# NorESMhub/BLOM

Hardware: AMD Instinct MI355X
Metric: simulated-days/sec (higher is better)
Workload: dtype f64; 1 GPU; channel 208x512x53 as 1 tile(s) of 208x512x53 along i, 1 tile per GPU, isopyc_bulkml/remap/geopotential/uc/enscon, ntr=3 (TKE, length-scale slot, ideal age: the reference default build), baclin=900s batrop=18s lstep=50; config 2's step (phy/mod_blom_step.F90:96-253: init_fluxes, tmsmt1, cmnfld2, difest_isobml [the whole routine: diffusivities estimated every step (NorESM defaults incl. rhsctp; the; physics=full, forcing=default, spinup_steps=0

## Files before the change

blom_amd/csrc/blomgpu_internal.h:

```cpp
#pragma once
#include <hip/hip_runtime.h>
#include <cstdint>
#include <string>
#include <unordered_map>
#include <vector>
#include "exp_libm.h"

#define NBDY 4

#ifdef BLOM_HOSTEMU
#define WAIT_VMCNT0() ((void)0)
#else
#define WAIT_VMCNT0() asm volatile("s_waitcnt vmcnt(0)" ::: "memory")
#endif

#define BLOM_REAL_FIELDS(X)                                                              \
                                                                          \
  X(u, 2 * K) X(v, 2 * K) X(dp, 2 * K) X(dpu, 2 * K) X(dpv, 2 * K) X(temp, 2 * K)        \
  X(saln, 2 * K) X(sigma, 2 * K) X(uflx, 2 * K) X(vflx, 2 * K) X(utflx, 2 * K)           \
  X(vtflx, 2 * K) X(usflx, 2 * K) X(vsflx, 2 * K)                                        \
  X(p, K + 1) X(pu, K + 1) X(pv, K + 1) X(phi, K + 1) X(cau, K) X(cav, K)                \
  X(ubflxs, 3) X(vbflxs, 3) X(ub, 2) X(vb, 2) X(pb, 2) X(pbu, 2) X(pbv, 2)               \
  X(ubflxs_p, 2) X(vbflxs_p, 2) X(pb_p, 1) X(pbu_p, 1) X(pbv_p, 1) X(ubcors_p, 1)        \
  X(vbcors_p, 1) X(sealv, 1)                                                             \
// ... 164 lines not shown
struct BtGlobal;
struct TileTable {
  int npx = 0, npy = 0, itdm = 0, nranks = 0;
  std::vector<int> i0, ii;
  std::vector<int> j0, jj;
  std::vector<int> rank;
  void ew_neighbours(int px, int py, bool periodic, int *west, int *east) const;
  bool tensor_product() const;
};
const char *tiletable_build(int npx, int npy, int itdm, int jtdm, const int *i0_pe, const int *ii_pe, const int *j0_pe,
                            const int *jj_pe, TileTable *out);
struct Tiling {
  int npx = 1, npy = 1;
  int px = 0, py = 0;
  const TileTable *tab = nullptr;
  TileGroup *group = nullptr;
  RcclComm *rccl = nullptr;
  bool multi() const { return npx * npy > 1 || rccl != nullptr; }
};

struct StepState {
  bool in_sequence = false;
  bool defer_checks = false;
  bool remap_handed_over = false;
  bool pbcor1_handed_over = false;
  bool pbcor2_handed_over = false;
  bool pbcor2_dp_in_wk = false;
  bool fluxes_lean = false;
  bool fluxes_zeroed = false;
  bool mom_early_done = false;
  bool convec_col_ahead = false;
  bool cmn_on_side = false;
  bool diapfl_mom_on_side = false, updtrc_on_side = false;
  bool pscan_done_ahead = false;
};

struct blomgpu_ctx {
  std::string expcnf = "channel";
  bool csdiag = false;
  int cnsvdi = 0;
  int cppm_compat = 1;
  int cppm_limiting = 2;
  int ale_method = 102, ale_upper_bndr_ord = 6, ale_lower_bndr_ord = 4, ale_tracer_limiting = 203, ale_velocity_limiting = 203;
  bool ale_tracer_pc_upper = true, ale_tracer_pc_lower = false, ale_velocity_pc_upper = true, ale_velocity_pc_lower = false;
  bool ale_density_pc_upper = false, ale_density_pc_lower = false;
  int ale_regrid_method = 2, ale_k_range_plevel = 1;
  double ale_regrid_nudge_ts = 86400., ale_stab_fac_limit = .75, ale_dpvar_fac = .75, ale_smooth_diff_max = 50000.;
  int ale_dktzu = 4, ale_dktzl = 2;
  double ale_dpmin_interior = .1 * 9806.;
  int ndiff_rec_per_face = 0;
  int ndiff_surface_align = 1;
  double rm0 = 1.2, rm5 = 0., niwgf = 0., niwbf = .35, niwlf = .5;
  std::string mlrttp = "constant";
  double trxday = 0., srxday = 0., trxdpt = 1., srxdpt = 1., trxlim = 1.5, srxlim = .5, sref = 34.65, area = 0., xmi = 0.;
  int lmi[5] = {11, 12, 1, 2, 3};
  bool aptflx = false, apsflx = false, ditflx = false, disflx = false, srxbal = false;
  int ntda = 0;
  double swamxd = 200., brine_mlbase_frac = 0.;
  int mlrmth = 1;
  double eddtra_ce = .06, tau_mlr = 86400., tau_growing_hbl = 300., tau_decaying_hbl = 86400., tau_growing_hml = 3600.,
         tau_decaying_hml = 259200., lfmin = 5.e3, mlbl_max_ratio = 3., eddtra_cl = .25, mstar = .5, nstar = .066, wpup_min = 1.e-3;
  double egc = 0., eggam = 200., eglsmn = 4000., egmndf = 0., egmxdf = 1500., egidfq = 1., rhiscf = 0., ri0 = 1.2, tkepf = 0.;
  double bdml_logc = 0.;
  int eddf2d = 0, edsprs = 1, edanis = 0, redi3d = 0, rhsctp = 0, edfsmo = 0;
  int edritp_opt = 2, edwmth_opt = 1;
  bool full_physics = false;
// ... 135 lines not shown
int st_xcsum(blomgpu_ctx *, const double *a, int itype, double *sum);
int st_xcsum_dev(blomgpu_ctx *, const double *a, int itype, int slot, double **sums_dev);
int st_thermf(blomgpu_ctx *, int m, int n, int mm, int nn, int k1m, int k1n);
int st_niw_ke_tendency(blomgpu_ctx *, int m, int mm);
int st_difest_isobml_pre(blomgpu_ctx *, int m, int n, int mm, int nn);
int st_difest_isobml(blomgpu_ctx *, int m, int n, int mm, int nn);
int st_budget_sums(blomgpu_ctx *, int ncall, int n, int nn);
int st_barotp(blomgpu_ctx *, int m, int n, int mm, int nn, int k1m, int k1n);
int st_eddtra(blomgpu_ctx *, int m, int n, int mm, int nn, int k1m, int k1n);
int st_eddtra_ale(blomgpu_ctx *, int m, int n, int mm, int nn, int k1m, int k1n);
int st_cppm(blomgpu_ctx *, int m, int n, int mm, int nn, int k1m, int k1n);
int st_init_cppm(blomgpu_ctx *);
int st_mxlayr_tail(blomgpu_ctx *, int nn, int k1n);
int ctx_err_words(blomgpu_ctx *);
int ctx_check_errors(blomgpu_ctx *);
int st_kfpla_halo(blomgpu_ctx *, int n);
int st_cmnfld1(blomgpu_ctx *, int m, int n, int mm, int nn, int k1m, int k1n);
int st_cmnfld2(blomgpu_ctx *, int m, int n, int mm, int nn, int k1m, int k1n);
int diapfl_column3_launch(blomgpu_ctx *, int n, int nn, int *errflag);
#define R_BASE(ntr) (8 + 3 * (ntr))
#define R_DP(ntr) (R_BASE(ntr) + 0)
#define R_T(ntr) (R_BASE(ntr) + 1)
#define R_S(ntr) (R_BASE(ntr) + 2)
#define R_TR(ntr, nt) (R_BASE(ntr) + 3 + (nt))
int st_ale_vdifft(blomgpu_ctx *, int m, int n, int mm, int nn, int k1m, int k1n);
int st_ale_vdiffm(blomgpu_ctx *, int m, int n, int mm, int nn, int k1m, int k1n);
int st_ale_forcing(blomgpu_ctx *, int m, int n, int mm, int nn, int k1m, int k1n);
int st_cmnfld_bfsqi_ale(blomgpu_ctx *, int m, int n, int mm, int nn, int k1m, int k1n);
int st_ale_regrid_remap(blomgpu_ctx *, int m, int n, int mm, int nn, int k1m, int k1n);
void ale_free(blomgpu_ctx *);
int ale_check_deferred(blomgpu_ctx *);
int st_mxlayr(blomgpu_ctx *, int m, int n, int mm, int nn, int k1m, int k1n);
int st_mom_pupv(blomgpu_ctx *, int off, int lo, int hi);
int st_convec_velocity(blomgpu_ctx *, int nn);
int launch_dpudpv(blomgpu_ctx *, int off, int flags);
int remap_tile_launch(blomgpu_ctx *, int n, int mm, int nn, int tsel, bool fold);
int pbcor_tile_launch(blomgpu_ctx *, int which, int m, int offc, int offf, int from_remap);
int launch_pscan(blomgpu_ctx *, int off, int lo, int hi_off);
int st_xctilr(blomgpu_ctx *, double *base, int l1, int ld, int mh, int nh, int itype);
int st_xctilr_arctic_multi(blomgpu_ctx *, int nf, double *const *ptrs, const int *nlevs, const int *mhs, const int *nhs,
                           const int *itypes);
int st_xctilr_multi(blomgpu_ctx *, int nf, double *const *ptrs, const int *nlevs, int mh, int nh, const int *itypes);
int st_crc(blomgpu_ctx *, const double *base, int nlev, int itype, unsigned *crc);
int st_crc_strips(blomgpu_ctx *, double *base, int nlev, int itype, unsigned *out, int cap, int *l0, int *ns);
int ctx_locate_ptr(const blomgpu_ctx *, const double *p, size_t *offset);
int rccl_xctilr(blomgpu_ctx *, double *base, int nlev, int mhl, int nhl);
int rccl_barotp_replicated(blomgpu_ctx *, int m, int n, int mm, int nn, int k1m, int k1n);
blomgpu_ctx *bt_global_ctx(const blomgpu_ctx *);
struct RcclLanded {
  const double *from_west = nullptr, *from_east = nullptr;
  int has_w = 0, has_e = 0, per = 0, mhl = 0, nhl = 0, nlev = 0;
  double *send_west = nullptr, *send_east = nullptr;
  int prepacked = 0;
};
int rccl_xctilr_multi_ex(blomgpu_ctx *, double *const *fields, int nf, int nlev, int mhl, int nhl, RcclLanded *landed);
int rccl_xctilr_multi(blomgpu_ctx *, double *const *fields, int nf, int nlev, int mhl, int nhl);

__device__ inline void xcd_block(unsigned &bx, unsigned &by) {
  const unsigned gx = gridDim.x, n = gx * gridDim.y;
  const unsigned lin = blockIdx.y * gx + blockIdx.x;
  const unsigned x = lin & 7u, s = lin >> 3;
  const unsigned q = n >> 3, r = n & 7u;
  const unsigned nl = x * q + (x < r ? x : r) + s;
  bx = nl % gx;
  by = nl / gx;
}

// ... 18 lines not shown
```

blom_amd/csrc/stage_barotp.hip:

```cpp
#include "blomgpu_internal.h"

#define ONEM 9806.

#define THREAD_IJ(V)                                                       \
  const int t_ = blockIdx.x * blockDim.x + threadIdx.x;                    \
  if (t_ >= (V).nplane) return;                                            \
  const int i = t_ % (V).ni - (NBDY - 1), j = t_ / (V).ni - (NBDY - 1);    \
  const size_t c = t_

__global__ void k_bt_bounds(const DevView *__restrict__ Vp, int m, int nn) {
  const DevView &V = *Vp;
  THREAD_IJ(V);
  if (j < 1 || j > V.jj || i < 1 || i > V.ii) return;
  const size_t np = V.nplane, om = c + (size_t)(m - 1) * np;
  if (V.m[I_iu][c]) {
    const double pbu = V.f[F_pbu][om];
    V.f[F_uglue][c] = V.P.cwbdts * exp_libm(1. - pbu / (V.P.cwbdls * ONEM));
    double mx = 0., mn = 0.;
    for (int k0 = 0; k0 < V.kk; k0 += COLUMN_U) {
      double a0[COLUMN_U];
#pragma unroll
      for (int q = 0; q < COLUMN_U; q++) a0[q] = V.f[F_u][c + (size_t)((k0 + q < V.kk ? k0 + q : V.kk - 1) + nn) * np];
#pragma unroll
      for (int q = 0; q < COLUMN_U; q++)
// ... 243 lines not shown
  const int i = t % V.ni - (NBDY - 1), j = t / V.ni - (NBDY - 1);
  if (i < 0 || i > V.ii + 1 || j < V.jj || j > V.jj + 2) return;
  const size_t c = t, on = (size_t)(n - 1) * V.nplane;
  double q = V.f[F_umaxb][c]; V.f[F_umaxb][c] = V.f[F_uminb][c]; V.f[F_uminb][c] = q;
  q = V.f[F_xixp][c + on]; V.f[F_xixp][c + on] = V.f[F_xixm][c + on]; V.f[F_xixm][c + on] = q;
  const int ilo = V.itdm / 2 - V.i0 + 1;
  if (j > V.jj || i >= (ilo > 0 ? ilo : 0)) {
    q = V.f[F_vmaxb][c]; V.f[F_vmaxb][c] = V.f[F_vminb][c]; V.f[F_vminb][c] = q;
    q = V.f[F_xiyp][c + on]; V.f[F_xiyp][c + on] = V.f[F_xiym][c + on]; V.f[F_xiym][c + on] = q;
  }
}

int bt_pair_halo(blomgpu_ctx *c, int set);
bool bt_phase_usable(blomgpu_ctx *c);
int bt_phase_launch(blomgpu_ctx *c, int m, int n, int ml, int nl, double woa, double wob, double wna, double wnb, int lll0,
                    int last, int src, int *src_out, int *ml_out, int *nl_out);
int bt_phase_check(blomgpu_ctx *c);
int bt_overlap_usable(blomgpu_ctx *c);
int bt_block_mode(blomgpu_ctx *c);
int bt_block_launch(blomgpu_ctx *c, int mode, int m, int n, int ml, int nl, const int *ph_last, const double (*ph_w)[4], int src,
                    int *src_out, int *ml_out, int *nl_out);
int bt_pair_launch(blomgpu_ctx *c, int m, int n, int ml, int nl, const double *wo, const double *wm, const double *wn,
                   int do_odd, int do_even, int src, int tsel, RcclLanded *rim);
int bt_pair_halo_landed(blomgpu_ctx *c, int set, RcclLanded *landed);

int st_barotp_bounds(blomgpu_ctx *c, int m, int nn) {
  hipLaunchKernelGGL(k_bt_bounds, plane_grid(c->h, 1, 64), dim3(64), 0, c->stream, c->d, m, nn);
  return 0;
}
int st_barotp_on(blomgpu_ctx *c, int m, int n, int mm, int nn, int k1m, int k1n, bool with_bounds);
int st_barotp(blomgpu_ctx *c, int m, int n, int mm, int nn, int k1m, int k1n) {
  TimeScope ts(c, "barotp");
  if (c->tiling.rccl && c->bt_global) return rccl_barotp_replicated(c, m, n, mm, nn, k1m, k1n);
  return st_barotp_on(c, m, n, mm, nn, k1m, k1n, true);
}
int st_barotp_on(blomgpu_ctx *c, int m, int n, int mm, int nn, int k1m, int k1n, bool with_bounds) {
  (void)mm; (void)k1m; (void)k1n;
  const DevView &h = c->h;
  const size_t np = h.nplane;
  const int ii = h.ii, jj = h.jj, lstep = h.P.lstep;
  if (lstep < 2 || lstep % 2) return ctx_fail(c, "barotp: lstep must be even (phy/mod_time.F90:137-139)");
  const dim3 g = plane_grid(h), b(256);
  if (with_bounds) hipLaunchKernelGGL(k_bt_bounds, plane_grid(h, 1, 64), dim3(64), 0, c->stream, c->d, m, nn);
  hipLaunchKernelGGL(k_bt_pvtrop_old, g, b, 0, c->stream, c->d, n);
  hipLaunchKernelGGL(k_bt_pvtrop, g, b, 0, c->stream, c->d, n);
  struct { int f, lev, nh, it; } hl[] = {
      {F_uglue, 0, 2, 3}, {F_utotn, 0, 2, 13}, {F_umaxb, 0, 2, 3}, {F_uminb, 0, 2, 3},
      {F_vglue, 0, 2, 4}, {F_vtotn, 0, 2, 14}, {F_vmaxb, 0, 2, 4}, {F_vminb, 0, 2, 4},
      {F_pvtrop, n - 1, 3, 2}, {F_pgfxm, n - 1, 2, 13}, {F_xixp, n - 1, 2, 3}, {F_xixm, n - 1, 2, 3},
      {F_pgfym, n - 1, 2, 14}, {F_xiyp, n - 1, 2, 4}, {F_xiym, n - 1, 2, 4}};
  for (int nhw = 2; nhw <= 3; nhw++) {
    double *ptrs[16];
    int nl[16], it[16], nf = 0;
    for (auto &x : hl)
      if (x.nh == nhw) { ptrs[nf] = h.f[x.f] + (size_t)x.lev * np; nl[nf] = 1; it[nf] = x.it; nf++; }
    if (int rc = st_xctilr_multi(c, nf, ptrs, nl, 1, nhw, it)) return rc;
  }

  if (h.nreg == 2) hipLaunchKernelGGL(k_bt_arctic_swap, g, b, 0, c->stream, c->d, n);
  if (int rc = ctx_err_words(c)) return rc;
  c->bt_restart = true;
  int lll0 = 1, ml = 1, nl = 2, set = 0;
  double woa = 0., wob = 0., wna = 0., wnb = 0.;
  if (c->barotp_fused && h.nreg != 2 && bt_block_mode(c)) {
    int ph_last[5];
    double ph_w[5][4];
    for (int nb = 1; nb <= 5; nb++) {
// ... 145 lines not shown
```

blom_amd/csrc/stage_convec.hip:

```cpp
#include "blomgpu_internal.h"
#include "eos.h"
#include "diapfl_common.h"

#define PLANE_IJ(V)                                                        \
  unsigned bx_, by_;                                                       \
  xcd_block(bx_, by_);                                                     \
  const int t_ = bx_ * blockDim.x + threadIdx.x;                           \
  (void)by_;                                                               \
  if (t_ >= (V).nplane) return;                                            \
  const int i = t_ % (V).ni - (NBDY - 1), j = t_ / (V).ni - (NBDY - 1);    \
  const size_t c = t_;                                                     \
  (void)i; (void)j; (void)c

#define MAXTR 64
enum { CV_UN = 0 };

__global__ __launch_bounds__(64) void k_convec_column(const DevView *__restrict__ Vp, int n, int nn, int *errflag) {
  const DevView &V = *Vp;
  PLANE_IJ(V);
  if (j < 1 || j > V.jj || i < 1 || i > V.ii || !V.m[I_ip][c]) return;
  const int kk = V.kk, ntr = V.ntr;
  const size_t np = V.nplane;
  const double epsilp = 1.e-12;
  gd_t ttem = V.f[F_temp] + c + (size_t)nn * np - np, ssal = V.f[F_saln] + c + (size_t)nn * np - np;
  gd_t delp = V.f[F_dp] + c + (size_t)nn * np - np, dens = V.f[F_sigma] + c + (size_t)nn * np - np;
  gcd_t densr = V.f[F_sigmar] + c - np;
  gd_t trc = V.f[F_trc] + c + (size_t)nn * np - np;
  const size_t ntl = (size_t)2 * kk * np;
#define TT(k) ttem[(size_t)(k) * np]
#define SS(k) ssal[(size_t)(k) * np]
#define DP(k) delp[(size_t)(k) * np]
#define DN(k) dens[(size_t)(k) * np]
#define DR(k) densr[(size_t)(k) * np]
#define TR(nt, k) trc[(size_t)(nt) * ntl + (size_t)(k) * np]
  double tdps, sdps, dps, ttmp, stmp, dtmp, q = 0.;
// ... 141 lines not shown
        k = kmix;
        while (dn2 < DR(k)) {
          if (k == 3) break;
          k = k - 1;
        }
        mix_tracers(true, d2, kfpl, kmix, q, 2, k);
        dps = 0.;
        for (int kz = kfpl; kz <= kmix; kz++) {
          dps = dps + DP(kz);
          DP(kz) = 0.;
        }
        kfpl = k;
        TT(kfpl) = ttmp; SS(kfpl) = stmp; DN(kfpl) = dn2; DP(kfpl) = dps;
        for (k = kfpl + 1; k <= kmix; k++) {
          const double dr = DR(k);
          TT(k) = ttmp;
          DN(k) = dr;
          SS(k) = eosd::sofsig(V.P, dr, ttmp);
        }
      }
    }
  }
  *kfpla = kfpl;
  column_scan(V.f[F_p][c], delp + np, V.f[F_p] + c, np, kk);
#undef TT
#undef SS
#undef DP
#undef DN
#undef DR
#undef TR
}

template <int NSINGLE>
__global__ __launch_bounds__(64) void k_convec_velocity(const DevView *__restrict__ Vp, int nn) {
  const DevView &V = *Vp;
  PLANE_IJ(V);
  if (j < 1 || j > V.jj || i < 1 || i > V.ii) return;
  const bool isv = by_ == 1;
  if (!V.m[isv ? I_iv : I_iu][c]) return;
  const int kk = V.kk;
  const size_t np = V.nplane, cm = isv ? c - V.ni : c - 1;
  gd_t vel = V.f[isv ? F_v : F_u] + c + (size_t)nn * np - np;
  gcd_t po = V.f[isv ? F_pv : F_pu] + c - np;
  gcd_t p = V.f[F_p] - np;
  gd_t un = WK(V, CV_UN + (isv ? 1 : 0)) + c - np;
  const double pbot = po[(size_t)(kk + 1) * np];
#define CV_U 8
#define CV_B 6
  int ko = 1;
  double po_lo = 0., po_hi = po[(size_t)2 * np];
  double v_cur = vel[(size_t)1 * np], v_nxt = vel[(size_t)(kk >= 2 ? 2 : 1) * np];
  double po_nx = kk >= 2 ? po[(size_t)3 * np] : 1.e300;
  double pn_lo = 0.;
  for (int k0 = 1; k0 <= kk; k0 += CV_U) {
    double a0[CV_U], a1[CV_U];
#pragma unroll
    for (int u = 0; u < CV_U; u++) {
      const int kq = k0 + u <= kk ? k0 + u : kk;
      a0[u] = p[c + (size_t)(kq + 1) * np]; a1[u] = p[cm + (size_t)(kq + 1) * np];
    }
#pragma unroll
    for (int u = 0; u < CV_U; u++) {
      const int kn = k0 + u;
      if (kn > kk) break;
      const double pn_hi = .5 * (fmin2(pbot, a0[u]) + fmin2(pbot, a1[u]));
      double r;
      if (pn_hi - pn_lo == 0.) {
        r = 0.;
      } else {
        double udpn = 0.;
        int nmv = 0;
        while (pn_hi > po_hi) {
          if (NSINGLE >= 1000 || nmv < NSINGLE) {
            nmv++;
            udpn = udpn + v_cur * (po_hi - fmax2(po_lo, pn_lo));
            ko = ko + 1;
            po_lo = po_hi;
            po_hi = ko <= kk ? po_nx : 1.e300;
            v_cur = v_nxt;
            v_nxt = vel[(size_t)(ko + 1 <= kk ? ko + 1 : kk) * np];
            po_nx = ko + 1 <= kk ? po[(size_t)(ko + 2) * np] : 1.e300;
          } else {
            double w[CV_B], q[CV_B];
#pragma unroll
            for (int b = 0; b < CV_B; b++) {
              const int kv = ko + 2 + b;
              w[b] = vel[(size_t)(kv <= kk ? kv : kk) * np];
              q[b] = po[(size_t)(kv <= kk ? kv + 1 : kk + 1) * np];
            }
#pragma unroll
            for (int b = 0; b < CV_B; b++)
              if (pn_hi > po_hi) {
                udpn = udpn + v_cur * (po_hi - fmax2(po_lo, pn_lo));
                ko = ko + 1;
                po_lo = po_hi;
                po_hi = ko <= kk ? po_nx : 1.e300;
                v_cur = v_nxt;
                v_nxt = w[b];
                po_nx = ko + 1 <= kk ? q[b] : 1.e300;
              }
          }
        }
        r = (udpn + v_cur * (pn_hi - fmax2(po_lo, pn_lo))) / (pn_hi - pn_lo);
      }
      un[(size_t)kn * np] = r;
      pn_lo = pn_hi;
    }
  }
  for (int k0 = 1; k0 <= kk; k0 += CV_U) {
    double a0[CV_U];
#pragma unroll
    for (int u = 0; u < CV_U; u++) a0[u] = un[(size_t)(k0 + u <= kk ? k0 + u : kk) * np];
#pragma unroll
    for (int u = 0; u < CV_U; u++)
      if (k0 + u <= kk) vel[(size_t)(k0 + u) * np] = a0[u];
  }
}

#define CVF_W 6
__global__ __launch_bounds__(64) void k_convec_velocity_flat(const DevView *__restrict__ Vp, int nn) {
  const DevView &V = *Vp;
  PLANE_IJ(V);
  __shared__ double s_pn[CVF_W][64], s_vel[CVF_W][64], s_po[CVF_W][64];
  if (j < 1 || j > V.jj || i < 1 || i > V.ii) return;
  const bool isv = by_ == 1;
  if (!V.m[isv ? I_iv : I_iu][c]) return;
  const int kk = V.kk, ln = threadIdx.x;
  const size_t np = V.nplane, cm = isv ? c - V.ni : c - 1;
  gd_t vel = V.f[isv ? F_v : F_u] + c + (size_t)nn * np - np;
  gcd_t po = V.f[isv ? F_pv : F_pu] + c - np;
  gcd_t p = V.f[F_p] - np;
  gd_t un = WK(V, CV_UN + (isv ? 1 : 0)) + c - np;
  const double pbot = po[(size_t)(kk + 1) * np];
  int ko = 1, of = 2, so_r = 2 % CVF_W, so_w = 2 % CVF_W;
  double po_lo = 0., po_hi = po[(size_t)2 * np], v_cur = vel[(size_t)1 * np], v_nx = 0., q_nx = 0.;
  bool hv_o = false;
  int kn = 1, nf = 1, sn_r = 1 % CVF_W, sn_w = 1 % CVF_W;
  double pn_lo = 0., pn_hi = 0., udpn = 0.;
  bool hv_n = false;
  while (kn <= kk) {
    if (__any(!hv_n || !hv_o)) {
      double a0[CVF_W], a1[CVF_W], w[CVF_W], q[CVF_W];
#pragma unroll
      for (int b = 0; b < CVF_W; b++) {
        const int lv = nf + b <= kk ? nf + b : kk, m = of + b <= kk ? of + b : kk;
        a0[b] = p[c + (size_t)(lv + 1) * np]; a1[b] = p[cm + (size_t)(lv + 1) * np];
        w[b] = vel[(size_t)m * np]; q[b] = po[(size_t)(m + 1) * np];
      }
// ... 45 lines not shown
    for (int u = 0; u < CV_U; u++) a0[u] = un[(size_t)(k0 + u <= kk ? k0 + u : kk) * np];
#pragma unroll
    for (int u = 0; u < CV_U; u++)
      if (k0 + u <= kk) vel[(size_t)(k0 + u) * np] = a0[u];
  }
}

__global__ void k_convec_dpudpv(const DevView *__restrict__ Vp, int nn) {
  const DevView &V = *Vp;
  unsigned bx_, by_;
  xcd_block(bx_, by_);
  const int t_ = bx_ * blockDim.x + threadIdx.x;
  if (t_ >= V.nplane) return;
  const int i = t_ % V.ni - (NBDY - 1), j = t_ / V.ni - (NBDY - 1);
  if (j < 1 || j > V.jj || i < 1 || i > V.ii) return;
  const size_t c = t_;
  const int k = by_;
  const size_t np = V.nplane, o0 = (size_t)k * np, o1 = (size_t)(k + 1) * np, ob = (size_t)V.kk * np;
  gcd_t p = V.f[F_p];
  if (V.m[I_iu][c]) {
    const size_t w = c - 1;
    const double q = fmin2(p[c + ob], p[w + ob]);
    V.f[F_dpu][c + (size_t)(k + nn) * np] =
        .5 * ((fmin2(q, p[w + o1]) - fmin2(q, p[w + o0])) + (fmin2(q, p[c + o1]) - fmin2(q, p[c + o0])));
  }
  if (V.m[I_iv][c]) {
    const size_t s = c - V.ni;
    const double q = fmin2(p[c + ob], p[s + ob]);
    V.f[F_dpv][c + (size_t)(k + nn) * np] =
        .5 * ((fmin2(q, p[s + o1]) - fmin2(q, p[s + o0])) + (fmin2(q, p[c + o1]) - fmin2(q, p[c + o0])));
  }
}

int st_convec_velocity(blomgpu_ctx *c, int nn) {
  switch (c->convec_nsingle) {
    case -1: hipLaunchKernelGGL(k_convec_velocity_flat, plane_grid(c->h, 2, 64), dim3(64), 0, c->stream, c->d, nn); break;
    case 0: hipLaunchKernelGGL(k_convec_velocity<0>, plane_grid(c->h, 2, 64), dim3(64), 0, c->stream, c->d, nn); break;
    case 1: hipLaunchKernelGGL(k_convec_velocity<1>, plane_grid(c->h, 2, 64), dim3(64), 0, c->stream, c->d, nn); break;
    case 2: hipLaunchKernelGGL(k_convec_velocity<2>, plane_grid(c->h, 2, 64), dim3(64), 0, c->stream, c->d, nn); break;
    case 3: hipLaunchKernelGGL(k_convec_velocity<3>, plane_grid(c->h, 2, 64), dim3(64), 0, c->stream, c->d, nn); break;
    default: hipLaunchKernelGGL(k_convec_velocity<1000>, plane_grid(c->h, 2, 64), dim3(64), 0, c->stream, c->d, nn); break;
  }
  HIPCHK(c, hipGetLastError());
  return 0;
}

int st_convec_column_ahead(blomgpu_ctx *c, int n, int nn) {
  const DevView &h = c->h;
  c->seq.convec_col_ahead = false;
  if (h.ntr > MAXTR || h.P.vcoord_tag != 1) return 0;
  if (int rc = ctx_err_words(c)) return rc;
  if (int rc = ctx_side_fork(c, 2)) return rc;
  hipLaunchKernelGGL(k_convec_column, plane_grid(h, 1, 64), dim3(64), 0, c->side, c->d, n, nn, c->err_dev + 3);
  HIPCHK(c, hipGetLastError());
  if (int rc = ctx_side_done(c, 3)) return rc;
  c->seq.convec_col_ahead = true;
  return 0;
}

int st_convec(blomgpu_ctx *c, int m, int n, int mm, int nn, int k1m, int k1n) {
  (void)m; (void)mm; (void)k1m; (void)k1n;
  const DevView &h = c->h;
  if (h.ntr > MAXTR) return ctx_fail(c, "convec: too many tracers for the device kernels");
  if (h.P.vcoord_tag != 1) return ctx_fail(c, "convec is only called for isopyc_bulkml (phy/mod_blom_step.F90:172-176)");
  if (int rc = ctx_err_words(c)) return rc;
  {
    TimeScope ts(c, "convec");
    if (c->seq.convec_col_ahead) {
      c->seq.convec_col_ahead = false;
      if (int rc = ctx_side_join(c, 3)) return rc;
    } else
      hipLaunchKernelGGL(k_convec_column, plane_grid(h, 1, 64), dim3(64), 0, c->stream, c->d, n, nn, c->err_dev + 3);
    if (int rc = st_xctilr(c, h.f[F_p], 1, h.kk + 1, 1, 1, 1)) return rc;
    if (int rc = st_convec_velocity(c, nn)) return rc;
    hipLaunchKernelGGL(k_convec_dpudpv, plane_grid(h, h.kk), dim3(256), 0, c->stream, c->d, nn);
  }
  HIPCHK(c, hipGetLastError());
  return 0;
}
```

blom_amd/csrc/stage_diapfl.hip:

```cpp
#include "blomgpu_internal.h"
#include "eos.h"

#define GRAV 9.806
#define ALPHA0 1.e-3
#define EPSILP 1.e-12
#define ONEM 9806.

#define THREAD_IJ(V)                                                       \
  unsigned bx_, by_;                                                       \
  xcd_block(bx_, by_);                                                     \
  const int t_ = bx_ * blockDim.x + threadIdx.x;                           \
  (void)by_;                                                               \
  if (t_ >= (V).nplane) return;                                            \
  const int i = t_ % (V).ni - (NBDY - 1), j = t_ / (V).ni - (NBDY - 1);    \
  const size_t c = t_

#define AR(slot, k) WK(V, slot)[c + (size_t)((k)-1) * np]

#include "diapfl_common.h"

__global__ void k_diapfl_kming(const DevView *__restrict__ Vp) {
  const DevView &V = *Vp;
  THREAD_IJ(V);
  if (j < 0 || j > V.jj + 1 || i < 0 || i > V.ii + 1 || !V.m[I_ip][c]) return;
// ... 126 lines not shown
  }
  const double ub = uprev;
  for (int k0 = kmax + 1; k0 <= kk; k0 += 2 * MU_) {
    double b0[2 * MU_], b1[2 * MU_];
#pragma unroll
    for (int u = 0; u < 2 * MU_; u++) {
      const int kq = k0 + u <= kk ? k0 + u : kk;
      b0[u] = p[mns + (size_t)(kq - 1) * np]; b1[u] = LV(p, kq);
    }
#pragma unroll
    for (int u = 0; u < 2 * MU_; u++)
      if (k0 + u <= kk && fmin2(b0[u], b1[u]) < pzb) LV(vel, k0 + u) = ub;
  }
}

__global__ void k_diapfl_dpudpv(const DevView *__restrict__ Vp, int nn) {
  const DevView &V = *Vp;
  THREAD_IJ(V);
  const int k = by_;
  const size_t np = V.nplane, o0 = (size_t)k * np, o1 = (size_t)(k + 1) * np, ob = (size_t)V.kk * np;
  gcd_t p = V.f[F_p];
  if (V.m[I_iu][c] && j >= 1 && j <= V.jj && i >= 1 && i <= V.ii + 1) {
    const size_t w = c - 1;
    const double q = fmin2(p[c + ob], p[w + ob]);
    V.f[F_dpu][c + (size_t)(k + nn) * np] = .5 * ((fmin2(q, p[w + o1]) - fmin2(q, p[w + o0])) + (fmin2(q, p[c + o1]) - fmin2(q, p[c + o0])));
  }
  if (V.m[I_iv][c] && j >= 1 && j <= V.jj + 1 && i >= 1 && i <= V.ii) {
    const size_t s = c - V.ni;
    const double q = fmin2(p[c + ob], p[s + ob]);
    V.f[F_dpv][c + (size_t)(k + nn) * np] = .5 * ((fmin2(q, p[s + o1]) - fmin2(q, p[s + o0])) + (fmin2(q, p[c + o1]) - fmin2(q, p[c + o0])));
  }
}

int st_diapfl(blomgpu_ctx *c, int n, int nn, int k1n) {
  (void)k1n;
  const DevView &h = c->h;
  if (h.P.vcoord_tag != 1) return ctx_fail(c, "diapfl is only called for isopyc_bulkml (phy/mod_blom_step.F90:172-186)");
  if (int rc = ctx_err_words(c)) return rc;
  int *errflag = c->err_dev + 0;
  {
    TimeScope ts(c, "diapfl");
    if (int rc = diapfl_column3_launch(c, n, nn, errflag)) return rc;
    {
      double *ptrs[4] = {h.f[F_p], h.f[F_fpug], h.f[F_fplg], h.f[F_util1]};
      const int nl[4] = {h.kk + 1, h.kk, h.kk, 1}, it[4] = {1, 1, 1, 1};
      if (int rc = st_xctilr_multi(c, 4, ptrs, nl, 1, 1, it)) return rc;
    }
    hipLaunchKernelGGL(k_diapfl_kming, plane_grid(h), dim3(256), 0, c->stream, c->d);
    const bool aside = ctx_overlap_on(c) && (c->phys_dag & 2) && !c->tiling.multi() && c->full_physics;
    hipStream_t s = c->stream;
    if (aside) {
      if (int rc = ctx_side_fork(c, 6)) return rc;
      s = c->side;
    }
    hipLaunchKernelGGL(k_diapfl_momentum, plane_grid(h, 2, 64), dim3(64), 0, s, c->d, nn);
    if (!c->seq.in_sequence || c->full_physics) hipLaunchKernelGGL(k_diapfl_dpudpv, plane_grid(h, h.kk), dim3(256), 0, s, c->d, nn);
    if (aside) {
      if (int rc = ctx_side_done(c, 7)) return rc;
      c->seq.diapfl_mom_on_side = true;
    }
  }
  HIPCHK(c, hipGetLastError());
  if (!c->seq.defer_checks) return ctx_check_errors(c);
  return 0;
}
```

blom_amd/csrc/stage_momtum.hip:

```cpp
#include "blomgpu_internal.h"

#include "momtum_common.h"

#define THREAD_IJ(V)                                                       \
  unsigned bx_, by_;                                                       \
  xcd_block(bx_, by_);                                                     \
  const int t_ = bx_ * blockDim.x + threadIdx.x;                           \
  (void)by_;                                                               \
  if (t_ >= (V).nplane) return;                                            \
  const int i = t_ % (V).ni - (NBDY - 1), j = t_ / (V).ni - (NBDY - 1);    \
  const size_t c = t_

#define S2_DRAG 3
#define S2_QUM 4


__global__ void k_mom_pupv(const DevView *__restrict__ Vp, int off, int lo, int hi, int ring) {
  const DevView &V = *Vp;
  THREAD_IJ(V);
  if (j < lo || j > V.jj + hi || i < lo || i > V.ii + hi) return;
  if (ring && j >= 1 && j <= V.jj && i >= 1 && i <= V.ii) return;
  const size_t np = V.nplane;
  if (V.m[I_iu][c]) column_scan(V.f[F_pu][c], V.f[F_dpu] + (size_t)off * np + c, V.f[F_pu] + c, np, V.kk);
  if (V.m[I_iv][c]) column_scan(V.f[F_pv][c], V.f[F_dpv] + (size_t)off * np + c, V.f[F_pv] + c, np, V.kk);
}

__global__ void k_mom_pscan(const DevView *__restrict__ Vp, int off, int lo, int hi, int ring) {
  const DevView &V = *Vp;
  THREAD_IJ(V);
  if (j < lo || j > V.jj + hi || i < lo || i > V.ii + hi || !V.m[I_ip][c]) return;
  if (ring && j >= 1 && j <= V.jj && i >= 1 && i <= V.ii) return;
  const size_t np = V.nplane;
  column_scan(V.f[F_p][c], V.f[F_dp] + (size_t)off * np + c, V.f[F_p] + c, np, V.kk);
}

__global__ void k_mom_drag(const DevView *__restrict__ Vp, int n, int nn) {
  const DevView &V = *Vp;
  THREAD_IJ(V);
  if (j < 0 || j > V.jj || i < 0 || i > V.ii || !V.m[I_ip][c]) return;
  const size_t np = V.nplane, on = (size_t)(n - 1) * np, e = c + 1, nb = c + V.ni;
  const double thkbop = THKBOT * ONEM, tsfac = V.P.dlt / V.P.delt1;
  gcd_t p = V.f[F_p];
  const double pbot = p[c + (size_t)V.kk * np];
  double u1 = 0., u2 = 0.;
  for (int k = 0; k < V.kk; k++) {
    const size_t okn = (size_t)(k + nn) * np;
    const double pbotl = fmax2(p[c + (size_t)(k + 1) * np], pbot - thkbop);
    const double ptopl = fmax2(p[c + (size_t)k * np], pbot - thkbop);
    u1 = u1 + (V.f[F_u][c + okn] + V.f[F_u][e + okn]) * (pbotl - ptopl);
    u2 = u2 + (V.f[F_v][c + okn] + V.f[F_v][nb + okn]) * (pbotl - ptopl);
  }
  V.f[F_util1][c] = u1;
  V.f[F_util2][c] = u2;
  gcd_t ubf = V.f[F_ubflxs_p] + on, vbf = V.f[F_vbflxs_p] + on, pbu = V.f[F_pbu] + on, pbv = V.f[F_pbv] + on;
  const double ubot = (ubf[c] / fmax2(EPSILPL, pbu[c] * V.f[F_scuy][c]) + ubf[e] / fmax2(EPSILPL, pbu[e] * V.f[F_scuy][e])) * tsfac +
                      u1 / thkbop;
  const double vbot = (vbf[c] / fmax2(EPSILPL, pbv[c] * V.f[F_scvx][c]) + vbf[nb] / fmax2(EPSILPL, pbv[nb] * V.f[F_scvx][nb])) * tsfac +
                      u2 / thkbop;
  const double ubbl = .5 * sqrt(ubot * ubot + vbot * vbot);
  const double q = V.P.cb * (ubbl + V.P.cbar);
  WK2(V, S2_DRAG)[c] = q * GRAV / (ALPHA0 * thkbop);
  V.f[F_ustarb][c] = sqrt(q * ubbl);
}


__global__ void k_mom_qplanes(const DevView *__restrict__ Vp, int m, int n) {
  const DevView &V = *Vp;
  THREAD_IJ(V);
  (void)i; (void)j;
  const size_t np = V.nplane, om = (size_t)(m - 1) * np, on = (size_t)(n - 1) * np;
  const double tsfac = V.P.dlt / V.P.delt1;
  gd_t q = WK2(V, S2_QUM);
  if (V.m[I_iu][c]) {
    const double sy = V.f[F_scuy][c];
    q[c] = V.f[F_ubflxs_p][c + om] * tsfac / (V.f[F_pbu][c + om] * sy);
    q[c + 2 * np] = V.f[F_ubflxs_p][c + on] * tsfac / (V.f[F_pbu][c + on] * sy);
  }
  if (V.m[I_iv][c]) {
    const double sx = V.f[F_scvx][c];
    q[c + np] = V.f[F_vbflxs_p][c + om] * tsfac / (V.f[F_pbv][c + om] * sx);
    q[c + 3 * np] = V.f[F_vbflxs_p][c + on] * tsfac / (V.f[F_pbv][c + on] * sx);
  }
}
// ... 3 lines not shown
  HIPCHK(c, hipGetLastError());
  return 0;
}

static int momtum_visc_chain(blomgpu_ctx *c, int m, int n, int mm, int nn) {
  const DevView &h = c->h;
  hipLaunchKernelGGL(k_mom_pupv, plane_grid(h, 1, 64), dim3(64), 0, c->stream, ctx_view(c, VIEW_MOM_A), mm, -1, 2, 0);
  hipLaunchKernelGGL(k_mom_qplanes, plane_grid(h, 1, 256), dim3(256), 0, c->stream, ctx_view(c, VIEW_MOM_A), m, n);
  return st_momtum_fused_layers(c, m, n, mm, nn, 1);
}

int st_momtum_early(blomgpu_ctx *c, int m, int n, int mm, int nn) {
  c->seq.mom_early_done = false;
  if (!ctx_overlap_on(c) || c->tiling.multi()) return 0;
  if (int rc = st_xctilr(c, c->h.f[F_difwgt], 1, 1, 2, 2, 1)) return rc;
  if (int rc = ctx_side_fork(c, 0)) return rc;
  hipStream_t main = c->stream;
  c->stream = c->side;
  const int rc = momtum_visc_chain(c, m, n, mm, nn);
  c->stream = main;
  if (rc) return rc;
  if (int rc2 = ctx_side_done(c, 1)) return rc2;
  c->seq.mom_early_done = true;
  return 0;
}

int st_momtum(blomgpu_ctx *c, int m, int n, int mm, int nn, int k1m, int k1n) {
  (void)k1m; (void)k1n;
  const DevView &h = c->h;
  const dim3 gcol = plane_grid(h, 1, 64), b64(64);
  if (ctx_overlap_on(c) && !c->tiling.multi())
    if (int rc = st_convec_column_ahead(c, n, nn)) return rc;
  TimeScope ts(c, "momtum");
  hipLaunchKernelGGL(k_mom_pscan, gcol, b64, 0, c->stream, ctx_view(c, VIEW_MOM_B), mm, -1, 2, 0);
  hipLaunchKernelGGL(k_mom_pscan, gcol, b64, 0, c->stream, c->d, mm, -1, 2, c->seq.in_sequence && h.P.vcoord_tag == 1 ? 1 : 0);
  hipLaunchKernelGGL(k_mom_pupv, gcol, b64, 0, c->stream, c->d, mm, -1, 2, 1);
  hipLaunchKernelGGL(k_mom_drag, gcol, b64, 0, c->stream, ctx_view(c, VIEW_MOM_B), n, nn);
  if (c->seq.mom_early_done) {
    c->seq.mom_early_done = false;
    if (int rc = ctx_side_join(c, 1)) return rc;
  } else {
    if (int rc = st_xctilr(c, h.f[F_difwgt], 1, 1, 2, 2, 1)) return rc;
    if (int rc = momtum_visc_chain(c, m, n, mm, nn)) return rc;
  }
  return st_momtum_fused_layers(c, m, n, mm, nn, 2);
}
```

blom_amd/csrc/stage_mxlayr.hip:

```cpp
#include "blomgpu_internal.h"
#include "eos.h"
#include "diapfl_common.h"
#include "exp_libm.h"

#define GRAV 9.806
#define ALPHA0 1.e-3
#define SPCIFH 3.99e3
#define EPSILP 1.e-12
#define ONEM 9806.
#define TENCM 980.6
#define ONECM 98.06
#define ONEMM 9.806
#define ONEMU 9.806e-3

#define PLANE_IJ(V)                                                        \
  unsigned bx_, by_;                                                       \
  xcd_block(bx_, by_);                                                     \
  const int t_ = bx_ * blockDim.x + threadIdx.x;                           \
  (void)by_;                                                               \
  if (t_ >= (V).nplane) return;                                            \
  const int i = t_ % (V).ni - (NBDY - 1), j = t_ / (V).ni - (NBDY - 1);    \
  const size_t c = t_;                                                     \
  (void)i; (void)j; (void)c

// ... 900 lines not shown
  const bool is_tke = nt >= 0 && P.itrtke >= 1 && nt + 1 == P.itrtke, is_gls = nt >= 0 && P.itrtke >= 1 && P.gls && nt + 1 == P.itrgls;
  if (is_tke || is_gls) {
    const double lo = is_tke ? TKE_MIN : GLS_PSI_MIN;
    for (int k0 = 1; k0 <= kk; k0 += 2 * COLUMN_U) {
      double a[2 * COLUMN_U];
#pragma unroll
      for (int u = 0; u < 2 * COLUMN_U; u++) a[u] = XX(k0 + u <= kk ? k0 + u : kk);
#pragma unroll
      for (int u = 0; u < 2 * COLUMN_U; u++)
        if (k0 + u <= kk && !(a[u] > lo)) XX(k0 + u) = fmax2(a[u], lo);
    }
    return;
  }
  gd_t corr = nt < 0 ? V.f[F_salt_corr] + c : V.f[F_trc_corr] + c + (size_t)nt * np;
  double tc = 0.;
  bool any = false;
  for (int k0 = 1; k0 <= kk; k0 += 2 * COLUMN_U) {
    double a[2 * COLUMN_U];
#pragma unroll
    for (int u = 0; u < 2 * COLUMN_U; u++) a[u] = XX(k0 + u <= kk ? k0 + u : kk);
#pragma unroll
    for (int u = 0; u < 2 * COLUMN_U; u++)
      if (k0 + u <= kk && a[u] < 0.) {
        if (!any) { tc = *corr; any = true; }
        tc = tc - fmin2(0., a[u]) * delp[(size_t)(k0 + u) * np] / GRAV;
        XX(k0 + u) = 0.;
      }
  }
  if (any) *corr = tc;
#undef XX
}

int st_mxlayr(blomgpu_ctx *c, int m, int n, int mm, int nn, int k1m, int k1n) {
  (void)m; (void)mm; (void)k1m;
  const DevView &h = c->h;
  if (h.P.vcoord_tag != 1) return ctx_fail(c, "mxlayr is only called for isopyc_bulkml (phy/mod_blom_step.F90:188-192)");
  if (h.ntr > MAXTR_MXL) return ctx_fail(c, "mxlayr: too many tracers for the device kernel");
  MxlPar M;
  if (c->mlrttp == "variable") M.rtsflg = 1;
  else if (c->mlrttp == "constant") M.rtsflg = 2;
  else if (c->mlrttp == "limited") M.rtsflg = 3;
  else return ctx_fail(c, " mlrttp = " + c->mlrttp + " is unsupported!");
  M.rm0 = c->rm0; M.rm5 = c->rm5; M.ce = c->eddtra_ce; M.rtau = 1. / c->tau_mlr; M.rlf = 1. / c->lfmin;
  M.niwgf = c->niwgf; M.niwbf = c->niwbf; M.swamxd = c->swamxd; M.mltmin = 5.; M.thktop = 10.;
  if (int rc = ctx_err_words(c)) return rc;
  M.maxitr_count = c->err_dev + 5;
  TimeScope ts(c, "mxlayr");
  hipLaunchKernelGGL(k_mxl_bg2_sig, plane_grid(h), dim3(256), 0, c->stream, c->d, nn);
  if (int rc = st_xctilr(c, h.f[F_util1], 1, 1, 1, 1, 1)) return rc;
  hipLaunchKernelGGL(k_mxl_bg2_grad, plane_grid(h), dim3(256), 0, c->stream, c->d);
  hipLaunchKernelGGL(k_mxl_bg2_sum, plane_grid(h), dim3(256), 0, c->stream, c->d);
  if (c->seq.diapfl_mom_on_side) {
    c->seq.diapfl_mom_on_side = false;
    if (int rc = ctx_side_join(c, 7)) return rc;
  }
  if (c->rm5 > 0.) {
    if (int rc = st_xctilr(c, h.f[F_u] + (size_t)(k1n - 1) * h.nplane, 1, h.kk, 1, 1, 13)) return rc;
    if (int rc = st_xctilr(c, h.f[F_v] + (size_t)(k1n - 1) * h.nplane, 1, h.kk, 1, 1, 14)) return rc;
  }
  hipLaunchKernelGGL(k_mxl_column, plane_grid(h, 1, 64), dim3(64), 0, c->stream, c->d, M, n, nn KPROF_PASS(3));
  const bool clamp_aside = ctx_overlap_on(c) && (c->phys_dag & 8) && !c->tiling.multi() && h.nreg != 2;
  if (clamp_aside)
    if (int rc = ctx_side_fork(c, 6)) return rc;
  hipLaunchKernelGGL(k_mxl_clamp, plane_grid(h, h.ntr + 1, 64), dim3(64), 0, clamp_aside ? c->side : c->stream, c->d, nn);
  HIPCHK(c, hipGetLastError());
  if (clamp_aside) c->seq.updtrc_on_side = true;
  if (int rc = st_mom_pupv(c, nn, 1, 0)) return rc;
  if (int rc = st_mxlayr_tail(c, nn, k1n)) return rc;
  return st_convec_velocity(c, nn);
}
```

Before: 1.597 simulated-days/sec.

## Fuse column scans, dpu/dpv, pu/pv and barotropic bounds into neighbouring kernels

Merges the momtum pressure scans, pu/pv scans and bottom-drag integral into one k_mom_front kernel. It also fuses dpu/dpv with the pu/pv scan in diapfl, folds the convec dpu/dpv computation into the convective velocity kernel, and computes the barotropic glue and max/min bounds inside that same kernel so st_barotp can skip k_bt_bounds. The goal is fewer kernel launches and fewer passes over the full 3D column data. In exchange, cross-stage state flags (diapfl_pupv_done, bt_bounds_done) now carry dependencies between stages, which is fragile if the stage order changes or fields are modified in between.

```diff
diff --git a/blom_amd/csrc/blomgpu_internal.h b/blom_amd/csrc/blomgpu_internal.h
--- a/blom_amd/csrc/blomgpu_internal.h
+++ b/blom_amd/csrc/blomgpu_internal.h
@@ -220,6 +220,8 @@
   bool convec_col_ahead = false;
   bool cmn_on_side = false;
   bool diapfl_mom_on_side = false, updtrc_on_side = false;
+  bool diapfl_pupv_done = false;
+  bool bt_bounds_done = false;
   bool pscan_done_ahead = false;
 };
 
@@ -421,7 +423,7 @@
 int ale_check_deferred(blomgpu_ctx *);
 int st_mxlayr(blomgpu_ctx *, int m, int n, int mm, int nn, int k1m, int k1n);
 int st_mom_pupv(blomgpu_ctx *, int off, int lo, int hi);
-int st_convec_velocity(blomgpu_ctx *, int nn);
+int st_convec_velocity(blomgpu_ctx *, int nn, int dpuv = 0, int bm = 0);
 int launch_dpudpv(blomgpu_ctx *, int off, int flags);
 int remap_tile_launch(blomgpu_ctx *, int n, int mm, int nn, int tsel, bool fold);
 int pbcor_tile_launch(blomgpu_ctx *, int which, int m, int offc, int offf, int from_remap);
diff --git a/blom_amd/csrc/stage_barotp.hip b/blom_amd/csrc/stage_barotp.hip
--- a/blom_amd/csrc/stage_barotp.hip
+++ b/blom_amd/csrc/stage_barotp.hip
@@ -299,7 +299,9 @@
 int st_barotp(blomgpu_ctx *c, int m, int n, int mm, int nn, int k1m, int k1n) {
   TimeScope ts(c, "barotp");
   if (c->tiling.rccl && c->bt_global) return rccl_barotp_replicated(c, m, n, mm, nn, k1m, k1n);
-  return st_barotp_on(c, m, n, mm, nn, k1m, k1n, true);
+  const bool have_bounds = c->seq.bt_bounds_done;
+  c->seq.bt_bounds_done = false;
+  return st_barotp_on(c, m, n, mm, nn, k1m, k1n, !have_bounds);
 }
 int st_barotp_on(blomgpu_ctx *c, int m, int n, int mm, int nn, int k1m, int k1n, bool with_bounds) {
   (void)mm; (void)k1m; (void)k1n;
diff --git a/blom_amd/csrc/stage_convec.hip b/blom_amd/csrc/stage_convec.hip
--- a/blom_amd/csrc/stage_convec.hip
+++ b/blom_amd/csrc/stage_convec.hip
@@ -1,6 +1,7 @@
 #include "blomgpu_internal.h"
 #include "eos.h"
 #include "diapfl_common.h"
+#include "exp_libm.h"
 
 #define PLANE_IJ(V)                                                        \
   unsigned bx_, by_;                                                       \
@@ -208,7 +209,7 @@
 }
 
 template <int NSINGLE>
-__global__ __launch_bounds__(64) void k_convec_velocity(const DevView *__restrict__ Vp, int nn) {
+__global__ __launch_bounds__(64) void k_convec_velocity(const DevView *__restrict__ Vp, int nn, int dpuv, int bm) {
   const DevView &V = *Vp;
   PLANE_IJ(V);
   if (j < 1 || j > V.jj || i < 1 || i > V.ii) return;
@@ -222,12 +223,19 @@
   gd_t un = WK(V, CV_UN + (isv ? 1 : 0)) + c - np;
   const double pbot = po[(size_t)(kk + 1) * np];
 #define CV_U 8
+#define ONEM_CV 9806.
 #define CV_B 6
   int ko = 1;
   double po_lo = 0., po_hi = po[(size_t)2 * np];
   double v_cur = vel[(size_t)1 * np], v_nxt = vel[(size_t)(kk >= 2 ? 2 : 1) * np];
   double po_nx = kk >= 2 ? po[(size_t)3 * np] : 1.e300;
   double pn_lo = 0.;
+  gd_t dz = V.f[isv ? F_dpv : F_dpu] + c + (size_t)nn * np - np;
+  double qz = 0., pc_lo = 0., pm_lo = 0.;
+  if (dpuv) {
+    qz = fmin2(p[c + (size_t)(kk + 1) * np], p[cm + (size_t)(kk + 1) * np]);
+    pc_lo = p[c + np]; pm_lo = p[cm + np];
+  }
   for (int k0 = 1; k0 <= kk; k0 += CV_U) {
     double a0[CV_U], a1[CV_U];
 #pragma unroll
@@ -239,6 +247,10 @@
     for (int u = 0; u < CV_U; u++) {
       const int kn = k0 + u;
       if (kn > kk) break;
+      if (dpuv) {
+        dz[(size_t)kn * np] = .5 * ((fmin2(qz, a1[u]) - fmin2(qz, pm_lo)) + (fmin2(qz, a0[u]) - fmin2(qz, pc_lo)));
+        pm_lo = a1[u]; pc_lo = a0[u];
+      }
       const double pn_hi = .5 * (fmin2(pbot, a0[u]) + fmin2(pbot, a1[u]));
       double r;
       if (pn_hi - pn_lo == 0.) {
@@ -283,13 +295,24 @@
       pn_lo = pn_hi;
     }
   }
+  double mx = 0., mn = 0.;
   for (int k0 = 1; k0 <= kk; k0 += CV_U) {
     double a0[CV_U];
 #pragma unroll
     for (int u = 0; u < CV_U; u++) a0[u] = un[(size_t)(k0 + u <= kk ? k0 + u : kk) * np];
 #pragma unroll
     for (int u = 0; u < CV_U; u++)
-      if (k0 + u <= kk) vel[(size_t)(k0 + u) * np] = a0[u];
+      if (k0 + u <= kk) {
+        vel[(size_t)(k0 + u) * np] = a0[u];
+        mx = fmax2(mx, a0[u]); mn = fmin2(mn, a0[u]);
+      }
+  }
+  if (bm) {
+    const double pbz = V.f[isv ? F_pbv : F_pbu][c + (size_t)(bm - 1) * np];
+    const double vmx = V.f[isv ? F_vmax : F_umax][c], sc = V.f[isv ? F_scvx : F_scuy][c];
+    V.f[isv ? F_vglue : F_uglue][c] = V.P.cwbdts * exp_libm(1. - pbz / (V.P.cwbdls * ONEM_CV));
+    V.f[isv ? F_vmaxb : F_umaxb][c] = (vmx - mx) * pbz * sc;
+    V.f[isv ? F_vminb : F_uminb][c] = (vmx + mn) * pbz * sc;
   }
 }
 
@@ -401,14 +424,19 @@
   }
 }
 
-int st_convec_velocity(blomgpu_ctx *c, int nn) {
+int st_barotp_bounds(blomgpu_ctx *c, int m, int nn);
+int st_convec_velocity(blomgpu_ctx *c, int nn, int dpuv, int bm) {
   switch (c->convec_nsingle) {
-    case -1: hipLaunchKernelGGL(k_convec_velocity_flat, plane_grid(c->h, 2, 64), dim3(64), 0, c->stream, c->d, nn); break;
-    case 0: hipLaunchKernelGGL(k_convec_velocity<0>, plane_grid(c->h, 2, 64), dim3(64), 0, c->stream, c->d, nn); break;
-    case 1: hipLaunchKernelGGL(k_convec_velocity<1>, plane_grid(c->h, 2, 64), dim3(64), 0, c->stream, c->d, nn); break;
-    case 2: hipLaunchKernelGGL(k_convec_velocity<2>, plane_grid(c->h, 2, 64), dim3(64), 0, c->stream, c->d, nn); break;
-    case 3: hipLaunchKernelGGL(k_convec_velocity<3>, plane_grid(c->h, 2, 64), dim3(64), 0, c->stream, c->d, nn); break;
-    default: hipLaunchKernelGGL(k_convec_velocity<1000>, plane_grid(c->h, 2, 64), dim3(64), 0, c->stream, c->d, nn); break;
+    case -1:
+      hipLaunchKernelGGL(k_convec_velocity_flat, plane_grid(c->h, 2, 64), dim3(64), 0, c->stream, c->d, nn);
+      if (dpuv) hipLaunchKernelGGL(k_convec_dpudpv, plane_grid(c->h, c->h.kk), dim3(256), 0, c->stream, c->d, nn);
+      if (bm) st_barotp_bounds(c, bm, nn);
+      break;
+    case 0: hipLaunchKernelGGL(k_convec_velocity<0>, plane_grid(c->h, 2, 64), dim3(64), 0, c->stream, c->d, nn, dpuv, bm); break;
+    case 1: hipLaunchKernelGGL(k_convec_velocity<1>, plane_grid(c->h, 2, 64), dim3(64), 0, c->stream, c->d, nn, dpuv, bm); break;
+    case 2: hipLaunchKernelGGL(k_convec_velocity<2>, plane_grid(c->h, 2, 64), dim3(64), 0, c->stream, c->d, nn, dpuv, bm); break;
+    case 3: hipLaunchKernelGGL(k_convec_velocity<3>, plane_grid(c->h, 2, 64), dim3(64), 0, c->stream, c->d, nn, dpuv, bm); break;
+    default: hipLaunchKernelGGL(k_convec_velocity<1000>, plane_grid(c->h, 2, 64), dim3(64), 0, c->stream, c->d, nn, dpuv, bm); break;
   }
   HIPCHK(c, hipGetLastError());
   return 0;
@@ -441,8 +469,7 @@
     } else
       hipLaunchKernelGGL(k_convec_column, plane_grid(h, 1, 64), dim3(64), 0, c->stream, c->d, n, nn, c->err_dev + 3);
     if (int rc = st_xctilr(c, h.f[F_p], 1, h.kk + 1, 1, 1, 1)) return rc;
-    if (int rc = st_convec_velocity(c, nn)) return rc;
-    hipLaunchKernelGGL(k_convec_dpudpv, plane_grid(h, h.kk), dim3(256), 0, c->stream, c->d, nn);
+    if (int rc = st_convec_velocity(c, nn, 1)) return rc;
   }
   HIPCHK(c, hipGetLastError());
   return 0;
diff --git a/blom_amd/csrc/stage_diapfl.hip b/blom_amd/csrc/stage_diapfl.hip
--- a/blom_amd/csrc/stage_diapfl.hip
+++ b/blom_amd/csrc/stage_diapfl.hip
@@ -182,6 +182,55 @@
   }
 }
 
+__global__ __launch_bounds__(64) void k_diapfl_dpudpv_pupv(const DevView *__restrict__ Vp, int nn) {
+  const DevView &V = *Vp;
+  THREAD_IJ(V);
+  const bool wu = V.m[I_iu][c] && j >= 1 && j <= V.jj && i >= 1 && i <= V.ii + 1;
+  const bool wv = V.m[I_iv][c] && j >= 1 && j <= V.jj + 1 && i >= 1 && i <= V.ii;
+  if (!wu && !wv) return;
+  const bool inner = j <= V.jj && i <= V.ii;
+  const int kk = V.kk;
+  const size_t np = V.nplane, w = c - 1, s = c - V.ni, bot = (size_t)kk * np;
+  gcd_t p = V.f[F_p];
+  const double pc_b = p[c + bot];
+  const double qu = wu ? fmin2(pc_b, p[w + bot]) : 0., qv = wv ? fmin2(pc_b, p[s + bot]) : 0.;
+  gd_t dpu = V.f[F_dpu] + (size_t)nn * np, dpv = V.f[F_dpv] + (size_t)nn * np, pug = V.f[F_pu], pvg = V.f[F_pv];
+  double pu = wu && inner ? pug[c] : 0., pv = wv && inner ? pvg[c] : 0.;
+  double pc0 = p[c], pw0 = wu ? p[w] : 0., ps0 = wv ? p[s] : 0.;
+  const size_t wl = wu ? w : c, sl = wv ? s : c;
+  for (int k0 = 0; k0 < kk; k0 += COLUMN_U) {
+    double a[COLUMN_U], b[COLUMN_U], d[COLUMN_U];
+#pragma unroll
+    for (int u = 0; u < COLUMN_U; u++) {
+      const size_t o1 = (size_t)((k0 + u < kk ? k0 + u : kk - 1) + 1) * np;
+      a[u] = p[c + o1]; b[u] = p[wl + o1]; d[u] = p[sl + o1];
+    }
+#pragma unroll
+    for (int u = 0; u < COLUMN_U; u++) {
+      const int k = k0 + u;
+      if (k < kk) {
+        const size_t o1 = (size_t)(k + 1) * np;
+        const double pc1 = a[u];
+        if (wu) {
+          const double pw1 = b[u];
+          const double dd = .5 * ((fmin2(qu, pw1) - fmin2(qu, pw0)) + (fmin2(qu, pc1) - fmin2(qu, pc0)));
+          dpu[c + (size_t)k * np] = dd;
+          if (inner) { pu = pu + dd; pug[c + o1] = pu; }
+          pw0 = pw1;
+        }
+        if (wv) {
+          const double ps1 = d[u];
+          const double dd = .5 * ((fmin2(qv, ps1) - fmin2(qv, ps0)) + (fmin2(qv, pc1) - fmin2(qv, pc0)));
+          dpv[c + (size_t)k * np] = dd;
+          if (inner) { pv = pv + dd; pvg[c + o1] = pv; }
+          ps0 = ps1;
+        }
+        pc0 = pc1;
+      }
+    }
+  }
+}
+
 int st_diapfl(blomgpu_ctx *c, int n, int nn, int k1n) {
   (void)k1n;
   const DevView &h = c->h;
@@ -204,7 +253,11 @@
       s = c->side;
     }
     hipLaunchKernelGGL(k_diapfl_momentum, plane_grid(h, 2, 64), dim3(64), 0, s, c->d, nn);
-    if (!c->seq.in_sequence || c->full_physics) hipLaunchKernelGGL(k_diapfl_dpudpv, plane_grid(h, h.kk), dim3(256), 0, s, c->d, nn);
+    if (c->seq.in_sequence && c->full_physics) {
+      hipLaunchKernelGGL(k_diapfl_dpudpv_pupv, plane_grid(h, 1, 64), dim3(64), 0, s, c->d, nn);
+      c->seq.diapfl_pupv_done = true;
+    } else if (!c->seq.in_sequence)
+      hipLaunchKernelGGL(k_diapfl_dpudpv, plane_grid(h, h.kk), dim3(256), 0, s, c->d, nn);
     if (aside) {
       if (int rc = ctx_side_done(c, 7)) return rc;
       c->seq.diapfl_mom_on_side = true;
diff --git a/blom_amd/csrc/stage_momtum.hip b/blom_amd/csrc/stage_momtum.hip
--- a/blom_amd/csrc/stage_momtum.hip
+++ b/blom_amd/csrc/stage_momtum.hip
@@ -25,30 +25,60 @@
   if (V.m[I_iv][c]) column_scan(V.f[F_pv][c], V.f[F_dpv] + (size_t)off * np + c, V.f[F_pv] + c, np, V.kk);
 }
 
-__global__ void k_mom_pscan(const DevView *__restrict__ Vp, int off, int lo, int hi, int ring) {
+__global__ __launch_bounds__(64) void k_mom_front(const DevView *__restrict__ Vp, double *__restrict__ pmod, int mm, int n, int nn, int ring_p) {
   const DevView &V = *Vp;
   THREAD_IJ(V);
-  if (j < lo || j > V.jj + hi || i < lo || i > V.ii + hi || !V.m[I_ip][c]) return;
-  if (ring && j >= 1 && j <= V.jj && i >= 1 && i <= V.ii) return;
+  if (j < -1 || j > V.jj + 2 || i < -1 || i > V.ii + 2) return;
   const size_t np = V.nplane;
-  column_scan(V.f[F_p][c], V.f[F_dp] + (size_t)off * np + c, V.f[F_p] + c, np, V.kk);
-}
-
-__global__ void k_mom_drag(const DevView *__restrict__ Vp, int n, int nn) {
-  const DevView &V = *Vp;
-  THREAD_IJ(V);
-  if (j < 0 || j > V.jj || i < 0 || i > V.ii || !V.m[I_ip][c]) return;
-  const size_t np = V.nplane, on = (size_t)(n - 1) * np, e = c + 1, nb = c + V.ni;
+  const int kk = V.kk;
+  const bool inner = j >= 1 && j <= V.jj && i >= 1 && i <= V.ii;
+  const bool wet = V.m[I_ip][c] != 0;
+  gcd_t dp = V.f[F_dp] + (size_t)mm * np + c;
+  double pbot = 0.;
+  if (wet) {
+    gd_t pa = V.f[F_p] + c, pm = (gd_t)pmod + c;
+    const bool tomod = !(ring_p && inner);
+    double acc = pa[0], accm = tomod ? pm[0] : 0.;
+    for (int k0 = 0; k0 < kk; k0 += COLUMN_U) {
+      double v[COLUMN_U];
+#pragma unroll
+      for (int u = 0; u < COLUMN_U; u++) v[u] = dp[(size_t)(k0 + u < kk ? k0 + u : kk - 1) * np];
+#pragma unroll
+      for (int u = 0; u < COLUMN_U; u++)
+        if (k0 + u < kk) {
+          acc = acc + v[u];
+          pa[(size_t)(k0 + u + 1) * np] = acc;
+          if (tomod) { accm = accm + v[u]; pm[(size_t)(k0 + u + 1) * np] = accm; }
+        }
+    }
+    pbot = acc;
+  }
+  if (!inner) {
+    if (V.m[I_iu][c]) column_scan(V.f[F_pu][c], V.f[F_dpu] + (size_t)mm * np + c, V.f[F_pu] + c, np, kk);
+    if (V.m[I_iv][c]) column_scan(V.f[F_pv][c], V.f[F_dpv] + (size_t)mm * np + c, V.f[F_pv] + c, np, kk);
+  }
+  if (!wet || j < 0 || j > V.jj || i < 0 || i > V.ii) return;
+  const size_t on = (size_t)(n - 1) * np, e = c + 1, nb = c + V.ni;
   const double thkbop = THKBOT * ONEM, tsfac = V.P.dlt / V.P.delt1;
-  gcd_t p = V.f[F_p];
-  const double pbot = p[c + (size_t)V.kk * np];
-  double u1 = 0., u2 = 0.;
-  for (int k = 0; k < V.kk; k++) {
-    const size_t okn = (size_t)(k + nn) * np;
-    const double pbotl = fmax2(p[c + (size_t)(k + 1) * np], pbot - thkbop);
-    const double ptopl = fmax2(p[c + (size_t)k * np], pbot - thkbop);
-    u1 = u1 + (V.f[F_u][c + okn] + V.f[F_u][e + okn]) * (pbotl - ptopl);
-    u2 = u2 + (V.f[F_v][c + okn] + V.f[F_v][nb + okn]) * (pbotl - ptopl);
+  gcd_t ug = V.f[F_u] + (size_t)nn * np, vg = V.f[F_v] + (size_t)nn * np;
+  double u1 = 0., u2 = 0., ptop = V.f[F_p][c];
+  for (int k0 = 0; k0 < kk; k0 += COLUMN_U) {
+    double d[COLUMN_U], a0[COLUMN_U], a1[COLUMN_U], b0[COLUMN_U], b1[COLUMN_U];
+#pragma unroll
+    for (int u = 0; u < COLUMN_U; u++) {
+      const size_t o = (size_t)(k0 + u < kk ? k0 + u : kk - 1) * np;
+      d[u] = dp[o]; a0[u] = ug[c + o]; a1[u] = ug[e + o]; b0[u] = vg[c + o]; b1[u] = vg[nb + o];
+    }
+#pragma unroll
+    for (int u = 0; u < COLUMN_U; u++)
+      if (k0 + u < kk) {
+        const double pk1 = ptop + d[u];
+        const double pbotl = fmax2(pk1, pbot - thkbop);
+        const double ptopl = fmax2(ptop, pbot - thkbop);
+        u1 = u1 + (a0[u] + a1[u]) * (pbotl - ptopl);
+        u2 = u2 + (b0[u] + b1[u]) * (pbotl - ptopl);
+        ptop = pk1;
+      }
   }
   V.f[F_util1][c] = u1;
   V.f[F_util2][c] = u2;
@@ -118,10 +148,8 @@
   if (ctx_overlap_on(c) && !c->tiling.multi())
     if (int rc = st_convec_column_ahead(c, n, nn)) return rc;
   TimeScope ts(c, "momtum");
-  hipLaunchKernelGGL(k_mom_pscan, gcol, b64, 0, c->stream, ctx_view(c, VIEW_MOM_B), mm, -1, 2, 0);
-  hipLaunchKernelGGL(k_mom_pscan, gcol, b64, 0, c->stream, c->d, mm, -1, 2, c->seq.in_sequence && h.P.vcoord_tag == 1 ? 1 : 0);
-  hipLaunchKernelGGL(k_mom_pupv, gcol, b64, 0, c->stream, c->d, mm, -1, 2, 1);
-  hipLaunchKernelGGL(k_mom_drag, gcol, b64, 0, c->stream, ctx_view(c, VIEW_MOM_B), n, nn);
+  hipLaunchKernelGGL(k_mom_front, gcol, b64, 0, c->stream, ctx_view(c, VIEW_MOM_B), h.f[F_p], mm, n, nn,
+                     c->seq.in_sequence && h.P.vcoord_tag == 1 ? 1 : 0);
   if (c->seq.mom_early_done) {
     c->seq.mom_early_done = false;
     if (int rc = ctx_side_join(c, 1)) return rc;
diff --git a/blom_amd/csrc/stage_mxlayr.hip b/blom_amd/csrc/stage_mxlayr.hip
--- a/blom_amd/csrc/stage_mxlayr.hip
+++ b/blom_amd/csrc/stage_mxlayr.hip
@@ -956,7 +956,7 @@
 }
 
 int st_mxlayr(blomgpu_ctx *c, int m, int n, int mm, int nn, int k1m, int k1n) {
-  (void)m; (void)mm; (void)k1m;
+  (void)mm; (void)k1m;
   const DevView &h = c->h;
   if (h.P.vcoord_tag != 1) return ctx_fail(c, "mxlayr is only called for isopyc_bulkml (phy/mod_blom_step.F90:188-192)");
   if (h.ntr > MAXTR_MXL) return ctx_fail(c, "mxlayr: too many tracers for the device kernel");
@@ -989,7 +989,11 @@
   hipLaunchKernelGGL(k_mxl_clamp, plane_grid(h, h.ntr + 1, 64), dim3(64), 0, clamp_aside ? c->side : c->stream, c->d, nn);
   HIPCHK(c, hipGetLastError());
   if (clamp_aside) c->seq.updtrc_on_side = true;
-  if (int rc = st_mom_pupv(c, nn, 1, 0)) return rc;
+  if (c->seq.diapfl_pupv_done) c->seq.diapfl_pupv_done = false;
+  else if (int rc = st_mom_pupv(c, nn, 1, 0)) return rc;
   if (int rc = st_mxlayr_tail(c, nn, k1n)) return rc;
-  return st_convec_velocity(c, nn);
-}
+  const bool bounds = c->seq.in_sequence && !c->tiling.multi();
+  if (int rc = st_convec_velocity(c, nn, 0, bounds ? m : 0)) return rc;
+  c->seq.bt_bounds_done = bounds;
+  return 0;
+}
```

New measurement: 1.621 simulated-days/sec, median of 6. +1.5%, better.
